# line/Human-Interaction-Generation

Measured on AMD Instinct MI355X. Metric: denoiser-fwd frames/s @ B=64·T=196, higher is better.
Workload: dtype f32; 1 GPU; MotionTransformer forward incl. the per-call cross-attention text side, BASELINE config 2: B=64/GPU T=196 F=150 d=512 L=8 H=8 ff=1024 N=77 Lt=256, linear attention, text embeddings supplied (CLIP stubbed); parallelism=dp1

## Files before the change

human-interaction-generation_amd/csrc/gemm.hip:

```cpp
#include <stdlib.h>

#include "hig_common.h"
#include "hig_host.h"

typedef float f32x16 __attribute__((ext_vector_type(16)));
typedef float f32x4 __attribute__((ext_vector_type(4)));
#ifndef HIG_GEMM_NT
#define HIG_GEMM_NT 0
#endif
#ifndef HIG_GEMM_SETPRIO
#define HIG_GEMM_SETPRIO 1
#endif
#ifndef HIG_GEMM_LDS_EPI
#define HIG_GEMM_LDS_EPI 1
#endif

namespace {

constexpr int BK = 32;
constexpr int NTHREADS = 256;
constexpr int RC_LD = BK + 4;
constexpr int BF_LD = BK + 8;
typedef __bf16 bf16x8 __attribute__((ext_vector_type(8)));
typedef __bf16 bf16x4 __attribute__((ext_vector_type(4)));
// ... 800 lines not shown
      } else {
        a.xsum = g.xcolsum;
      }
    }
  }
  auto al16 = [](const void* p) { return (reinterpret_cast<uintptr_t>(p) & 15) == 0; };
  a.vecx = (g.ldx % 4 == 0) && al16(g.X);
  a.vecy = (g.ldy % 4 == 0) && al16(g.Y);
  a.vecc = (a.g.ldc % 4 == 0) && al16(a.g.C) && (a.slab % 4 == 0) &&
           (!g.res || ((g.ldr % 4 == 0) && al16(g.res))) &&
           (!g.aux || ((g.ldaux % 4 == 0) && al16(g.aux)));
  constexpr int kStage = ((X_RS ? BK * BI : BI * RC_LD) + (Y_RS ? BK * BJ : BJ * RC_LD));
  constexpr int kLdsF32 = 2 * kStage * 4;
  constexpr int kLdsBf3 = 2 * (BI + BJ) * (BF_LD / 2) * 2 * 4;
  const int lds_bytes = (g.prec == HIG_PREC_BF16X3 && !X_RS && !Y_RS) ? kLdsBf3 : kLdsF32;
  int per_cu = 160 * 1024 / lds_bytes;
  per_cu = per_cu < 1 ? 1 : (per_cu > 8 ? 8 : per_cu);
  const int max_vgpr_blocks = (BI * BJ >= 128 * 128) ? 2 : 4;
  if (per_cu > max_vgpr_blocks) per_cu = max_vgpr_blocks;
  const bool fast = hig_gemm32_fast(g);
  if (tail_s > 1) {
    const int rem = a.ntiles % hig_chip_cus();
    a.tail_s = tail_s;
    a.tail_rem = rem;
    a.nmain = a.ntiles - rem;
    a.tail_chunk = g.R / tail_s;
    a.tail_ws = g_tail.ws;
    a.tail_cnt = g_tail.cnt;
    a.ntiles = a.nmain + rem * tail_s;
  }
  int gridx = hig_chip_cus() * per_cu;
  if (gridx > a.ntiles) gridx = a.ntiles;
  bool served = false;
  if constexpr (X_RS && Y_RS && XF == HIG_XF_NONE && EPI == HIG_EPI_NONE) {
    if (splits > 1 && a.g.C == slabs) {
      const int rc = hig_wgrad_wsp32_try(g, splits, slabs, a.slab, a.xsum, a.xsum_stride, st);
      if (rc < 0) return rc;
      served = rc == HIG_OK;
    }
  }
  if (!served && a.ntiles > 0 && g.R >= 0) {
    hig_gemm_path_count(a.tail_s > 1 ? HIG_GEMM_PATH_TAIL32 : splits > 1 ? HIG_GEMM_PATH_SPLIT32 : HIG_GEMM_PATH_TILED32);
    bool launched = false;
    if constexpr (!X_RS && !Y_RS) {
      if (fast && g.prec == HIG_PREC_BF16X3) {
        hipLaunchKernelGGL((gemm_f32_kernel<BI, BJ, X_RS, Y_RS, XF, XF_ON_Y, EPI, true, HIG_PREC_BF16X3>),
                           dim3(gridx, splits), dim3(NTHREADS), 0, st, a);
        launched = true;
      } else if (fast && g.prec == HIG_PREC_BF16) {
        hipLaunchKernelGGL((gemm_f32_kernel<BI, BJ, X_RS, Y_RS, XF, XF_ON_Y, EPI, true, HIG_PREC_BF16>),
                           dim3(gridx, splits), dim3(NTHREADS), 0, st, a);
        launched = true;
      }
    }
    if (!launched) {
      if (fast)
        hipLaunchKernelGGL((gemm_f32_kernel<BI, BJ, X_RS, Y_RS, XF, XF_ON_Y, EPI, true, HIG_PREC_F32>),
                           dim3(gridx, splits), dim3(NTHREADS), 0, st, a);
      else
        hipLaunchKernelGGL((gemm_f32_kernel<BI, BJ, X_RS, Y_RS, XF, XF_ON_Y, EPI, false, HIG_PREC_F32>),
                           dim3(gridx, splits), dim3(NTHREADS), 0, st, a);
    }
  }
  HIG_CHECK_LAUNCH();
  if (splits > 1) {
    const int64_t n4 = (int64_t)g.I * g.J / 4;
    const int64_t want = (n4 + 255) / 256;
    const int blocks = (int)(want > 2048 ? 2048 : want);
    hipLaunchKernelGGL(reduce_slabs_kernel, dim3(blocks), dim3(256), 0, st, slabs, splits, a.slab, n4, g.C,
                       a.xsum ? n4 + g.I / 4 : (int64_t)0, a.xsum ? g.xcolsum : (float*)nullptr, se);
    HIG_CHECK_LAUNCH();
  }
  return HIG_OK;
}

template <bool X_RS, bool Y_RS, int XF, bool XF_ON_Y, int EPI>
int launch_sized(const hig_gemm_desc& g, int splits, float* slabs, int64_t slab, hipStream_t st, const SplitEpilogue& se, int variant) {
  const int tile = splits > 1 ? (wgrad_tile(g.I, g.J, g.prec) == 128 ? 0 : 3) : variant % 16, tail_s = splits > 1 ? 1 : variant / 16;
  switch (tile) {
    case 0: return launch<128, 128, X_RS, Y_RS, XF, XF_ON_Y, EPI>(g, splits, slabs, slab, st, se, tail_s);
    case 1: return launch<64, 128, X_RS, Y_RS, XF, XF_ON_Y, EPI>(g, splits, slabs, slab, st, se, tail_s);
    case 2: return launch<128, 64, X_RS, Y_RS, XF, XF_ON_Y, EPI>(g, splits, slabs, slab, st, se, tail_s);
    default: return launch<64, 64, X_RS, Y_RS, XF, XF_ON_Y, EPI>(g, splits, slabs, slab, st, se, tail_s);
  }
}

}

namespace {
int gemm_dispatch(const hig_gemm_desc& g, int splits, float* slabs, hipStream_t st, const SplitEpilogue& se);
}
int hig_chip_cus() {
  static int cache[64];
  int dev = 0;
  if (hipGetDevice(&dev) != hipSuccess || dev < 0 || dev >= 64) return 256;
  int v = __atomic_load_n(&cache[dev], __ATOMIC_RELAXED);
  if (v == 0) {
    if (hipDeviceGetAttribute(&v, hipDeviceAttributeMultiprocessorCount, dev) != hipSuccess || v <= 0) v = 256;
    static const int forced = getenv("HIG_CHIP_CUS") ? atoi(getenv("HIG_CHIP_CUS")) : 0;
    if (forced > 0) v = forced;
    __atomic_store_n(&cache[dev], v, __ATOMIC_RELAXED);
  }
  return v;
}

int hig_reduce_slabs(const float* slabs, int splits, int64_t slab, int64_t n, float* out, hipStream_t st) {
  const int64_t n4 = n / 4;
  const int64_t want = (n4 + 255) / 256;
  const int blocks = (int)(want > 2048 ? 2048 : (want < 1 ? 1 : want));
  hipLaunchKernelGGL(reduce_slabs_kernel, dim3(blocks), dim3(256), 0, st, slabs, splits, slab, n4, out, (int64_t)0,
                     (float*)nullptr, SplitEpilogue{nullptr, nullptr, 0, 1});
  HIG_CHECK_LAUNCH();
  return HIG_OK;
}

int hig_gemm_launch(const hig_gemm_desc& g, int splits, float* slabs, hipStream_t st) {
  return gemm_dispatch(g, splits, slabs, st, SplitEpilogue{nullptr, nullptr, 0, 1});
}
void hig_gemm_set_tail_scratch(void* ws, int64_t bytes) {
  if (!ws || bytes <= HIG_GEMM_TAIL_CNT_BYTES || (reinterpret_cast<uintptr_t>(ws) & 15)) {
    g_tail = TailScratch{nullptr, nullptr, 0};
    return;
  }
  g_tail.cnt = static_cast<unsigned*>(ws);
  g_tail.ws = reinterpret_cast<float*>(static_cast<char*>(ws) + HIG_GEMM_TAIL_CNT_BYTES);
  g_tail.ws_bytes = bytes - HIG_GEMM_TAIL_CNT_BYTES;
}
namespace {
int gemm_dispatch(const hig_gemm_desc& g, int splits, float* slabs, hipStream_t st, const SplitEpilogue& se) {
  const hig_plan p = hig_gemm32_plan(g, g_tail.ws ? g_tail.ws_bytes : 0, hig_gemm_switch_values(), hig_chip_cus());
  if (p.rc != HIG_OK) return hig_set_error(p.rc, "%s", p.msg);
  if (p.launches == 0) return HIG_OK;
  const int64_t slab = (int64_t)g.I * g.J;
  if (splits > 1) HIG_REQUIRE(slabs && g.epi == HIG_EPI_NONE && slab % 4 == 0 && g.ldc == g.J,
                              "hig_gemm: split-R needs slabs, EPI_NONE, dense C");
  if (splits <= 1 && p.path == HIG_GEMM_PATH_WSP32) {
    if (p.launches == 1) return hig_gemm_wsp32_launch(g, p.variant, st);
    hig_gemm_desc p1, p2;
    hig_gemm32_two_pass(g, &p1, &p2);
    HIG_TRY(hig_gemm_wsp32_launch(p1, p.variant, st));
    return hig_gemm_wsp32_launch(p2, HIG_WSP_VARIANT(0, 0), st);
  }
#define CASE(xrs, yrs, xfv, ony, epiv)                                                   \
  if (g.x_rs == xrs && g.y_rs == yrs && g.xf == xfv && (g.xf == HIG_XF_NONE || g.xf_on_y == ony) && \
      g.epi == epiv)                                                                     \
    return launch_sized<xrs, yrs, xfv, ony, epiv>(g, splits, slabs, slab, st, se, p.variant);
  HIG_GEMM32_COMBOS(CASE)
#undef CASE
  return hig_set_error(HIG_EUNSUPPORTED, "hig_gemm: combination x_rs=%d y_rs=%d xf=%d on_y=%d epi=%d not built",
                       g.x_rs, g.y_rs, g.xf, g.xf_on_y, g.epi);
}
}

int hig_gemm_few_rows(const hig_gemm_desc& g, float* scratch, int64_t scratch_floats, hipStream_t st) {
  const int enabled = hig_gemm_switch_values().few_rows_split;
  const int64_t out = (int64_t)g.I * g.J;
  const bool ok = enabled && scratch && g.I > 0 && g.I <= 64 && g.x_rs == 0 && g.y_rs == 0 && g.ldc == g.J && g.J % 4 == 0 &&
                  (g.epi == HIG_EPI_BIAS || g.epi == HIG_EPI_BIAS_RES) && g.bias &&
                  (g.xf == HIG_XF_NONE || g.xf == HIG_XF_SILU) && g.R % 32 == 0 &&
                  (reinterpret_cast<uintptr_t>(g.bias) & 15) == 0 && (reinterpret_cast<uintptr_t>(g.C) & 15) == 0 &&
                  (g.epi != HIG_EPI_BIAS_RES || (g.res && (reinterpret_cast<uintptr_t>(g.res) & 15) == 0 && g.ldr % 4 == 0));
  int splits = 1;
  if (ok) {
    const int64_t tiles = (g.J + 63) / 64;
    int64_t s = 1024 / tiles;
    if (s > g.R / 64) s = g.R / 64;
    if (s > 16) s = 16;
    if (s * out > scratch_floats) s = scratch_floats / out;
    splits = (int)(s < 1 ? 1 : s);
  }
  if (splits <= 1) return hig_gemm_launch(g, 1, nullptr, st);
  hig_gemm_desc p = g;
  p.epi = HIG_EPI_NONE;
  p.bias = nullptr;
  p.res = nullptr;
  return gemm_dispatch(p, splits, scratch, st,
                       SplitEpilogue{g.bias, g.epi == HIG_EPI_BIAS_RES ? g.res : nullptr, g.ldr, g.J / 4});
}

extern "C" int hig_gemm(const hig_gemm_desc* g, hig_stream_t stream) {
  HIG_REQUIRE(g, "hig_gemm: null descriptor");
  HIG_REQUIRE(g->prec == HIG_PREC_F32 || g->prec == HIG_PREC_BF16X3 || g->prec == HIG_PREC_BF16,
              "hig_gemm: unknown prec %d", g->prec);
  return hig_gemm_launch(*g, 1, nullptr, hig_stream(stream));
}

extern "C" int hig_gemm_debug_stamps(void* buf) {
  g_gemm_stamps = static_cast<unsigned long long*>(buf);
  return HIG_OK;
}

extern "C" int64_t hig_gemm_tail_ws_bytes(void) { return HIG_GEMM_TAIL_BYTES; }

static long long g_path_launches[HIG_GEMM_NPATHS];
void hig_gemm_path_count(int path) {
  if (path >= 0 && path < HIG_GEMM_NPATHS) __atomic_fetch_add(&g_path_launches[path], 1, __ATOMIC_RELAXED);
}
extern "C" int64_t hig_gemm_path_launches(int32_t path) {
  if (path < 0 || path >= HIG_GEMM_NPATHS) return -1;
  return __atomic_load_n(&g_path_launches[path], __ATOMIC_RELAXED);
}

extern "C" int hig_gemm_ws(const hig_gemm_desc* g, void* ws, int64_t ws_bytes, hig_stream_t stream) {
  HIG_REQUIRE(g, "hig_gemm_ws: null descriptor");
  HIG_REQUIRE(g->prec == HIG_PREC_F32 || g->prec == HIG_PREC_BF16X3 || g->prec == HIG_PREC_BF16,
              "hig_gemm_ws: unknown prec %d", g->prec);
  HIG_REQUIRE(!ws || (ws_bytes >= HIG_GEMM_TAIL_BYTES && (reinterpret_cast<uintptr_t>(ws) & 15) == 0),
              "hig_gemm_ws: scratch must be 16-byte aligned and hig_gemm_tail_ws_bytes() long");
  hig_gemm_set_tail_scratch(ws, ws_bytes);
  const int rc = hig_gemm_launch(*g, 1, nullptr, hig_stream(stream));
  hig_gemm_set_tail_scratch(nullptr, 0);
  return rc;
}

extern "C" int64_t hig_gemm_split_scratch_floats(const hig_gemm_desc* g, int32_t splits) {
  if (!g || g->I <= 0 || g->J <= 0) return -1;
  const int64_t per = (int64_t)g->I * g->J + g->I;
  const int64_t cap = splits > 0 ? splits : (g->R / 256 > 1 ? g->R / 256 : 1);
  return per * cap;
}
extern "C" int hig_gemm_split(const hig_gemm_desc* g, int32_t splits, float* slabs, int64_t slab_floats,
                              hig_stream_t stream) {
  HIG_REQUIRE(g && slabs && splits >= 0, "hig_gemm_split: bad arguments");
  HIG_REQUIRE(g->prec == HIG_PREC_F32 || g->prec == HIG_PREC_BF16X3 || g->prec == HIG_PREC_BF16,
              "hig_gemm_split: unknown prec %d", g->prec);
  int s = splits > 0 ? splits : wgrad_splits(g->I, g->J, g->R, slab_floats, g->prec);
  HIG_REQUIRE((int64_t)s * ((int64_t)g->I * g->J + g->I) <= slab_floats, "hig_gemm_split: %d splits need %lld scratch floats, got %lld",
              s, (long long)((int64_t)s * ((int64_t)g->I * g->J + g->I)), (long long)slab_floats);
  return hig_gemm_launch(*g, s, slabs, hig_stream(stream));
}
```

human-interaction-generation_amd/csrc/hig_host.h:

```cpp
#pragma once
#include <stdlib.h>
#include <string.h>

#include <type_traits>

#include "hig_common.h"

int hig_gemm_launch(const hig_gemm_desc& g, int splits, float* slabs, hipStream_t st);
void hig_gemm_path_count(int path);
void hig_attn_path_count(int path, int split);
int hig_gemm_few_rows(const hig_gemm_desc& g, float* scratch, int64_t scratch_floats, hipStream_t st);

constexpr int64_t HIG_GEMM_TAIL_CNT_BYTES = 1024;
constexpr int64_t HIG_GEMM_TAIL_BYTES = HIG_GEMM_TAIL_CNT_BYTES + 256 * 16384;
void hig_gemm_set_tail_scratch(void* ws, int64_t bytes);

int hig_chip_cus();
inline int hig_chip_xcds() { const int c = hig_chip_cus() / 32; return c < 1 ? 1 : c; }

int hig_gemm16_launch(const hig_gemm16_desc& g, hipStream_t st);
int hig_gemm16_split_launch(const hig_gemm16_desc& g, int splits, float* slabs, int64_t slab_floats, hipStream_t st);
struct hig_wg_reduce {
  const float* slabs; int nsplit; int64_t slab;
  int64_t n4; float* out;
  int64_t nb4; float* dbias;
};
constexpr int HIG_WG_RB_MAX = 12;
int hig_wgrad16_launch(const void* dC, int64_t ldd, const void* act, int64_t ldx, int64_t rows, int J, int K, float* dW, float* dbias,
                       int splits, float* slabs, int64_t slab_floats, hipStream_t st, hig_wg_reduce* deferred = nullptr);
int hig_wgrad16_reduce_batch(const hig_wg_reduce* entries, int n, hipStream_t st);
struct hig_wg_problem {
  const void* dC; int64_t ldd; const void* act; int64_t ldx; int64_t rows; int J, K; float* dW; float* dbias; int splits;
};
constexpr int HIG_WG_GROUP_MAX = 4;
int hig_wgrad16_launch_group(const hig_wg_problem* probs, int n, float* slabs, int64_t slab_floats, hipStream_t st, hig_wg_reduce* deferred,
                             int64_t* used_floats);
int64_t hig_wgrad16_rule_floats(int64_t rows, int J, int K, int64_t room);
int hig_reduce_slabs(const float* slabs, int splits, int64_t slab, int64_t n, float* out, hipStream_t st);
struct hig_gemm_switches {
  int wsp16, ws16, ws_rows, ws_nwj, lnfold, lnfold1024, fewrow16, tile16;
  int wsp32, tile32, tail32;
  int few_rows_split;
};
const hig_gemm_switches& hig_gemm_switch_values();
struct hig_plan { int rc, path, launches, variant; char msg[256]; };
#define HIG_WSP_VARIANT(xt, aux) ((xt) + 4 * ((aux) ? 1 : 0))
#define HIG_WS16_VARIANT(nwj, role) ((nwj) + 256 * (role))
#define HIG_TILE16_VARIANT(rows, bk, ns) ((rows) * 1000 + (bk) * 10 + (ns))
#define HIG_TILE32_VARIANT(tile, tail) ((tile) + 16 * (tail))
hig_plan hig_gemm16_plan(const hig_gemm16_desc& g, const hig_gemm_switches& sw, int cus);
hig_plan hig_gemm32_plan(const hig_gemm_desc& g, int64_t tail_ws_bytes, const hig_gemm_switches& sw, int cus);
bool hig_gemm_ws16_lnfold_ok(int64_t rows, int d);
int hig_gemm_wsp16_launch(const hig_gemm16_desc& g, int variant, hipStream_t st);
int hig_gemm_ws16_launch(const hig_gemm16_desc& g, int variant, hipStream_t st);
int hig_gemm_wsp32_launch(const hig_gemm_desc& g, int variant, hipStream_t st);
constexpr int64_t HIG_GEMM_TAIL_UNIT_BYTES = 256 * 16 * 4;
constexpr int HIG_P32_MAXSEG = 3;
inline int hig_wsp32_segments(int np, int* seg_p0, int* seg_np) {
  int nseg = 0, p0 = 0;
  for (int s = 0; s < HIG_P32_MAXSEG; ++s) { seg_p0[s] = 0; seg_np[s] = 1; }
  while (np > 0) {
    int n = 256;
    while (n > np) n >>= 1;
    if (nseg == HIG_P32_MAXSEG) return -1;
    seg_p0[nseg] = p0; seg_np[nseg] = n; ++nseg;
    p0 += n; np -= n;
  }
  return nseg;
}
inline void hig_gemm32_two_pass(const hig_gemm_desc& g, hig_gemm_desc* p1, hig_gemm_desc* p2) {
  *p1 = g; p1->R = 1024;
  *p2 = g; p2->X = g.X + 1024; p2->Y = g.Y + 1024; p2->R = g.R - 1024;
  p2->epi = HIG_EPI_RES; p2->bias = nullptr; p2->res = g.C; p2->ldr = g.ldc;
}
inline bool hig_gemm32_fast(const hig_gemm_desc& g) {
  auto vec = [](const void* p, int64_t ld) { return ld % 4 == 0 && (reinterpret_cast<uintptr_t>(p) & 15) == 0; };
  return vec(g.X, g.ldx) && vec(g.Y, g.ldy) && g.R % 32 == 0 && g.R > 0 && (!g.x_rs || (g.I % 4 == 0 && g.I >= 4)) && (!g.y_rs || (g.J % 4 == 0 && g.J >= 4));
}
#ifdef HIG_GEMM_PROBE
#define HIG_GEMM32_COMBOS(CASE) CASE(0, 0, HIG_XF_NONE, 0, HIG_EPI_BIAS_GELU)
#else
#define HIG_GEMM32_COMBOS(CASE)                                                                                       \
                                                                                \
  CASE(0, 0, HIG_XF_NONE, 0, HIG_EPI_NONE) CASE(0, 0, HIG_XF_NONE, 0, HIG_EPI_BIAS) CASE(0, 0, HIG_XF_NONE, 0, HIG_EPI_BIAS_GELU) \
  CASE(0, 0, HIG_XF_NONE, 0, HIG_EPI_BIAS_POS) CASE(0, 0, HIG_XF_NONE, 0, HIG_EPI_BIAS_RES)                           \
  CASE(0, 0, HIG_XF_NONE, 0, HIG_EPI_RES)                                 \
  CASE(0, 0, HIG_XF_NONE, 0, HIG_EPI_DGELU) CASE(0, 0, HIG_XF_LN, 0, HIG_EPI_BIAS) CASE(0, 0, HIG_XF_LN_MOD_SILU, 0, HIG_EPI_BIAS_RES) \
  CASE(0, 0, HIG_XF_SILU, 0, HIG_EPI_BIAS) CASE(0, 0, HIG_XF_SILU, 0, HIG_EPI_BIAS_RES)                               \
  CASE(0, 0, HIG_XF_SILU, 0, HIG_EPI_NONE)                                 \
                                                                                             \
  CASE(0, 1, HIG_XF_NONE, 0, HIG_EPI_NONE) CASE(0, 1, HIG_XF_NONE, 0, HIG_EPI_RES) CASE(0, 1, HIG_XF_NONE, 0, HIG_EPI_DGELU) \
                                                                                      \
  CASE(1, 1, HIG_XF_NONE, 0, HIG_EPI_NONE) CASE(1, 1, HIG_XF_LN, 1, HIG_EPI_NONE) CASE(1, 1, HIG_XF_LN_MOD_SILU, 1, HIG_EPI_NONE) \
  CASE(1, 1, HIG_XF_SILU, 1, HIG_EPI_NONE)
#endif
template <int... E> struct hig_epi_list {};
using hig_epi16_fewrow = hig_epi_list<HIG_EPI_NONE, HIG_EPI_BIAS, HIG_EPI_BIAS_GELU, HIG_EPI_BIAS_RES, HIG_EPI_BIAS_SILU, HIG_EPI_BIAS_RES_SILU>;
using hig_epi16_all = hig_epi_list<HIG_EPI_NONE, HIG_EPI_BIAS, HIG_EPI_BIAS_GELU, HIG_EPI_BIAS_RES, HIG_EPI_BIAS_SILU, HIG_EPI_BIAS_RES_SILU, HIG_EPI_RES, HIG_EPI_DGELU>;
template <int... E, class F>
int hig_with_epi(hig_epi_list<E...>, int epi, int none, F&& f) {
  int rc = none;
  (void)(((epi == E) && ((rc = f(std::integral_constant<int, E>{})), true)) || ...);
  return rc;
}
struct hig_attn_switches {
  int apply_wave;
  int fullattn_waves;
  int fullattn_valu;
};
const hig_attn_switches& hig_attn_switch_values();
struct hig_attn_call {
  int entry, io;
  int B, rows, Tk, H, hd;
  bool has_scratch;
  int facts;
};
inline int hig_attn_facts(bool operands, uintptr_t in, uintptr_t out, uintptr_t par = 0, bool out_i32 = true) {
  return (operands ? HIG_ATTN_FACT_OPERANDS : 0) | ((in & 7) ? 0 : HIG_ATTN_FACT_IN8) | ((in & 15) ? 0 : HIG_ATTN_FACT_IN16) |
         ((out & 7) ? 0 : HIG_ATTN_FACT_OUT8) | ((out & 15) ? 0 : HIG_ATTN_FACT_OUT16) | ((par & 15) ? 0 : HIG_ATTN_FACT_PAR16) |
         (out_i32 ? HIG_ATTN_FACT_OUT_I32 : 0);
}
inline uintptr_t hig_low_bits(const void* p) { return reinterpret_cast<uintptr_t>(p); }
inline uintptr_t hig_low_bits(int64_t ld, int elem_bytes) { return (uintptr_t)ld * (uintptr_t)elem_bytes; }
struct hig_attn_plan_t { int rc, path, split, variant; char msg[160]; };
#define HIG_ATTN_VARIANT_MERGE 1
hig_attn_plan_t hig_attn_plan_for(const hig_attn_call& c, const hig_attn_switches& sw, int cus, bool big_lds_ok);
bool hig_attn_mfma_hd(int hd);
inline int hig_attn_plan_entry(hig_attn_plan_t* p, const hig_attn_call& c, bool big_lds_ok = true) {
  *p = hig_attn_plan_for(c, hig_attn_switch_values(), hig_chip_cus(), big_lds_ok);
  if (p->rc != HIG_OK) return hig_set_error(p->rc, "%s", p->msg);
  hig_attn_path_count(p->path, p->split);
  return HIG_OK;
}
struct hig_denoiser_switches {
  int32_t text_batch, text_fork, fwd_split, lnfold32, fwd16_fork, ctx16, joint16, fuse_apply, fuse_out, edge16, bwd_overlap;
};
static_assert(sizeof(hig_denoiser_switches) == HIG_DN_NSWITCHES * sizeof(int32_t), "one int32 per switch, in the documented order");
const hig_denoiser_switches& hig_denoiser_switch_values();
struct hig_denoiser_call {
  int entry;
  int B, T, F, d, E, ff, L, H, hd, N, nsty, two, full, prec;
  bool training, has_xf_out;
  int facts;
  bool capturing;
};
struct hig_denoiser_plan_t {
  int32_t entry;
  int32_t text_batched, text_fork, fuse_apply, fold32, split;
  int32_t fork_emb, fork_text, ctx_mm16, joint16, fuse_mm16, fuse_out;
  int32_t fuse_front;
  int32_t wgrad_fork;
  int32_t edge16, Fp;
  int32_t wants_side_stream;
};
static_assert(sizeof(hig_denoiser_plan_t) == HIG_DN_PLAN_NSLOTS * sizeof(int32_t), "one int32 per HIG_DN_PLAN_* slot");
hig_denoiser_plan_t hig_denoiser_plan_for(const hig_denoiser_call& c, const hig_denoiser_switches& sw, int cus, bool wsp32_active);
constexpr int HIG_MAX_TEXT_LAYERS = 32;
struct hig_edge16_offsets { int64_t dout, x, wot, dwo, dwj, dbo, end; };
inline hig_edge16_offsets hig_edge16_layout(int64_t M, int64_t Fp, int d) {
  auto up256 = [](int64_t v) { return (v + 255) / 256 * 256; };
  hig_edge16_offsets e;
  e.dout = 0;
  e.x = e.dout + up256(M * Fp * 2);
  e.wot = e.x + up256(M * Fp * 2);
// ... 146 lines not shown
```

include/hig.h:

```cpp
#ifndef HIG_H
#define HIG_H

#include <stddef.h>
#include <stdint.h>

#ifdef __cplusplus
extern "C" {
#endif

#define HIG_OK 0
#define HIG_EINVAL (-1)
#define HIG_EHIP (-2)
#define HIG_EUNSUPPORTED (-3)

#define HIG_ATTN_LINEAR 0
#define HIG_ATTN_FULL 1

#define HIG_PREC_F32 0
#define HIG_PREC_BF16X3 1
#define HIG_PREC_BF16 2

typedef void* hig_stream_t;

int hig_version(void);
// ... 191 lines not shown

int hig_denoiser_bwd(const hig_dims* dims, const void* const* params, const float* x,
                     const int64_t* t, const int64_t* length, const float* xf_out,
                     const void* textctx, const void* workspace, const float* dout,
                     void* const* grads, float* dx, float* dxf_proj, float* dxf_out,
                     void* bwd_workspace, hig_stream_t stream);
int64_t hig_bwd_workspace_bytes(const hig_dims* dims);
int hig_denoiser_bwd_hooked(const hig_dims* dims, const void* const* params, const float* x,
                            const int64_t* t, const int64_t* length, const float* xf_out,
                            const void* textctx, const void* workspace, const float* dout,
                            void* const* grads, float* dx, float* dxf_proj, float* dxf_out,
                            void* bwd_workspace, hig_stream_t stream, hig_layer_hook hook, void* hook_user,
                            hig_stream_t comm_stream);

typedef struct hig_text_dims {
  int32_t B, N, W;
  int32_t Lt, H, ff, L, E;
  int32_t prec;
} hig_text_dims;
enum {
  HIG_T_PRE_W = 0, HIG_T_PRE_B,
  HIG_T_LN_W, HIG_T_LN_B,
  HIG_T_PROJ_W, HIG_T_PROJ_B,
  HIG_T_NGLOBAL
};
enum {
  HIG_TL_IN_W = 0, HIG_TL_IN_B,
  HIG_TL_OUT_W, HIG_TL_OUT_B,
  HIG_TL_N1_W, HIG_TL_N1_B,
  HIG_TL_FF1_W, HIG_TL_FF1_B,
  HIG_TL_FF2_W, HIG_TL_FF2_B,
  HIG_TL_N2_W, HIG_TL_N2_B,
  HIG_TL_NLAYER
};
int64_t hig_text_head_workspace_bytes(const hig_text_dims* dims, int training);
int64_t hig_text_head_bwd_workspace_bytes(const hig_text_dims* dims);
int hig_text_head_fwd(const hig_text_dims* dims, const void* const* params, const float* clip_out,
                      const int64_t* eot, float* xf_out, float* xf_proj, void* workspace, int training,
                      hig_stream_t stream);
int hig_text_head_bwd(const hig_text_dims* dims, const void* const* params, const float* clip_out,
                      const int64_t* eot, const float* xf_out, const void* workspace, const float* dxf_out,
                      const float* dxf_proj, void* const* grads, float* dclip, void* bwd_workspace,
                      hig_stream_t stream);

enum { HIG_CD_B = 0, HIG_CD_N, HIG_CD_W, HIG_CD_H, HIG_CD_L, HIG_CD_VOCAB, HIG_CD_PREC, HIG_CD_NSLOTS };
enum {
  HIG_CT_TOK_EMB = 0,
  HIG_CT_POS_EMB,
  HIG_CT_LNF_W, HIG_CT_LNF_B,
  HIG_CT_NGLOBAL
};
enum {
  HIG_CTL_LN1_W = 0, HIG_CTL_LN1_B,
  HIG_CTL_IN_W, HIG_CTL_IN_B,
  HIG_CTL_OUT_W, HIG_CTL_OUT_B,
  HIG_CTL_LN2_W, HIG_CTL_LN2_B,
  HIG_CTL_FC_W, HIG_CTL_FC_B,
  HIG_CTL_PROJ_W, HIG_CTL_PROJ_B,
  HIG_CTL_NLAYER
};
int64_t hig_clip_text_workspace_bytes(const int32_t* dims);
int hig_clip_text_fwd(const int32_t* dims, const void* const* params, const int64_t* tokens, float* out,
                      void* workspace, hig_stream_t stream);
int hig_clip_embed(const float* tok_emb, const float* pos_emb, const int64_t* tokens, int32_t B, int32_t N, int32_t W,
                   int32_t vocab, float* out, int64_t ldo, hig_stream_t stream);
int hig_quick_gelu(float* x, int64_t n, hig_stream_t stream);
int hig_causal_attn_fwd(const float* Q, int64_t ldq, const float* K, const float* V, int64_t ldk, int32_t B, int32_t N,
                        int32_t H, float* Y, int64_t ldy, hig_stream_t stream);

typedef struct hig_eval_dims {
  int32_t B, T, F;
  int32_t d, H, ff, L;
  int32_t C;
  int32_t cls;
  int32_t prec;
} hig_eval_dims;
enum {
  HIG_EV_SEQ_EMB = 0,
  HIG_EV_JOINT1_W, HIG_EV_JOINT1_B,
  HIG_EV_JOINT2_W, HIG_EV_JOINT2_B,
  HIG_EV_OUT1_W, HIG_EV_OUT1_B,
  HIG_EV_OUT2_W, HIG_EV_OUT2_B,
  HIG_EV_HEAD_W, HIG_EV_HEAD_B,
  HIG_EV_CLS_IN,
  HIG_EV_NGLOBAL
};
int64_t hig_eval_encoder_workspace_bytes(const hig_eval_dims* dims);
int hig_eval_encoder_fwd(const hig_eval_dims* dims, const void* const* params, const float* x1,
                         const float* x2, const int64_t* length, float* logits, float* feature,
                         void* workspace, hig_stream_t stream);
int64_t hig_eval_encoder_train_workspace_bytes(const hig_eval_dims* dims);
int64_t hig_eval_encoder_bwd_workspace_bytes(const hig_eval_dims* dims);
int hig_eval_encoder_fwd_train(const hig_eval_dims* dims, const void* const* params, const float* x1,
                               const float* x2, const int64_t* length, float* logits, float* feature,
                               void* workspace, hig_stream_t stream);
int hig_eval_encoder_bwd(const hig_eval_dims* dims, const void* const* params, const float* x1, const float* x2,
                         const int64_t* length, const void* workspace, const float* dlogits,
                         const float* dfeature , void* const* grads, void* bwd_workspace,
                         hig_stream_t stream);
int hig_softmax_xent(const float* logits, const int64_t* labels, int32_t B, int32_t C, float* loss ,
                     float* dlogits, int64_t* pred, hig_stream_t stream);

int hig_gather_frames(const float* bank, const int64_t* seq_off, const int32_t* frame_ix,
                      const void* stats, int32_t stats_f64, int32_t rows, int32_t T, int32_t F,
                      float* out, hig_stream_t stream);

int hig_eval_pairs_build(const float* src, const int64_t* src_off, const int32_t* m_len, const int32_t* shift,
                         const int64_t* src_off_host, const int32_t* m_len_host, const int32_t* shift_host,
                         int64_t src_floats, int32_t N, int32_t F_in, int32_t F_out, int32_t T_out, float* out,
                         hig_stream_t stream);

int hig_recover_joints(const float* motion, const float* stats, int32_t rows, int32_t T, int32_t F,
                       int32_t joints, int32_t init_first, float* pos, hig_stream_t stream);


#define HIG_XF_NONE 0
#define HIG_XF_LN 1
#define HIG_XF_LN_MOD_SILU 2
#define HIG_XF_SILU 3
#define HIG_EPI_NONE 0
#define HIG_EPI_BIAS 1
#define HIG_EPI_BIAS_GELU 2
#define HIG_EPI_BIAS_RES 3
#define HIG_EPI_BIAS_POS 4
#define HIG_EPI_RES 5
#define HIG_EPI_DGELU 6
#define HIG_EPI_BIAS_SILU 7
#define HIG_EPI_BIAS_RES_SILU 8
typedef struct hig_gemm_desc {
  const float* X; int64_t ldx; int32_t x_rs;
  const float* Y; int64_t ldy; int32_t y_rs;
  float* C; int64_t ldc;
  int32_t I, J, R;
  int32_t xf, xf_on_y, epi, prec;
  const float* bias;
  const float* res; int64_t ldr;
  float* aux; int64_t ldaux;
  const float* stats;
  const float* gamma; const float* beta;
  const float* ss; int64_t ss_ld; int32_t ss_shift_off; int32_t rows_per_sample;
  const float* pos; int64_t ldpos; int32_t T;
  int32_t pos_shift;
  float* xcolsum;
  float* row_stats_out;
  const float* row_stats_in;
  const float* ln_colsum;
} hig_gemm_desc;
int hig_gemm(const hig_gemm_desc* g, hig_stream_t stream);
int64_t hig_gemm_tail_ws_bytes(void);
int hig_gemm_ws(const hig_gemm_desc* g, void* ws, int64_t ws_bytes, hig_stream_t stream);
int hig_gemm_debug_stamps(void* buf);
int64_t hig_gemm_split_scratch_floats(const hig_gemm_desc* g, int32_t splits);
int hig_gemm_split(const hig_gemm_desc* g, int32_t splits, float* slabs, int64_t slab_floats, hig_stream_t stream);

typedef struct hig_gemm16_desc {
  const void* X; int64_t ldx;
  const void* Y; int64_t ldy;
  void* C; int64_t ldc; int32_t c_f32;
  int32_t I, J, R;
  int32_t epi;
  const float* bias;
  const void* res; int64_t ldr; int32_t res_f32;
  float* row_stats_out;
  const float* row_stats_in;
  const float* ln_colsum;
  void* aux; int64_t ldaux;
} hig_gemm16_desc;
int hig_gemm_bf16(const hig_gemm16_desc* g, hig_stream_t stream);
int64_t hig_gemm_bf16_split_scratch_floats(const hig_gemm16_desc* g, int32_t splits);
int hig_gemm_bf16_split(const hig_gemm16_desc* g, int32_t splits, float* slabs, int64_t slab_floats, hig_stream_t stream);
int hig_gemm_bf16_debug_stamps(void* buf);
int hig_gemm_ws16_debug_stamps(void* buf);
int hig_gemm_wsp16_debug_stamps(void* buf);
int hig_gemm_wsp32_debug_stamps(void* buf);
int64_t hig_gemm_wsp32_launches(void);
#define HIG_GEMM_PATH_TILED32 0
#define HIG_GEMM_PATH_WSP32 1
#define HIG_GEMM_PATH_TAIL32 2
#define HIG_GEMM_PATH_WGRAD_WSP32 3
#define HIG_GEMM_PATH_SPLIT32 4
#define HIG_GEMM_PATH_WSP16 5
#define HIG_GEMM_PATH_WS16 6
#define HIG_GEMM_PATH_FEWROW16 7
#define HIG_GEMM_PATH_TILED16 8
#define HIG_GEMM_PATH_SPLIT16 9
#define HIG_GEMM_PATH_WGRAD16 10
#define HIG_GEMM_NPATHS 11
int64_t hig_gemm_path_launches(int32_t path);
int hig_gemm_bf16_plan(const hig_gemm16_desc* g, int32_t chip_cus, int32_t* path, int32_t* launches, int32_t* variant);
int hig_gemm_plan(const hig_gemm_desc* g, int32_t has_tail_scratch, int32_t chip_cus, int32_t* path, int32_t* launches, int32_t* variant);
int hig_gemm_bf16_lnfold_plan(int64_t rows, int32_t d, int32_t chip_cus);
#define HIG_ATTN_PATH_CTX 0
#define HIG_ATTN_PATH_CTX_MFMA 1
#define HIG_ATTN_PATH_CTX_PART 2
#define HIG_ATTN_PATH_APPLY 3
#define HIG_ATTN_PATH_APPLY_MFMA 4
#define HIG_ATTN_PATH_APPLY_WAVE64 5
#define HIG_ATTN_PATH_APPLY_STY 6
#define HIG_ATTN_PATH_APPLY_STY_WAVE64 7
#define HIG_ATTN_PATH_APPLY_BWD 8
#define HIG_ATTN_PATH_APPLY_BWD_MFMA 9
#define HIG_ATTN_PATH_CTX_BWD 10
#define HIG_ATTN_PATH_CTX_BWD_MFMA 11
#define HIG_ATTN_PATH_FULL_FWD 12
#define HIG_ATTN_PATH_FULL_FWD_MFMA 13
#define HIG_ATTN_PATH_FULL_BWD 14
#define HIG_ATTN_PATH_FULL_BWD_MFMA 15
#define HIG_ATTN_NPATHS 16
int64_t hig_attn_path_launches(int32_t path);
int32_t hig_attn_last_split(void);
#define HIG_ATTN_ENTRY_CTX 0
#define HIG_ATTN_ENTRY_APPLY 1
#define HIG_ATTN_ENTRY_APPLY_STY 2
#define HIG_ATTN_ENTRY_APPLY_BWD 3
#define HIG_ATTN_ENTRY_CTX_BWD 4
#define HIG_ATTN_ENTRY_FULL_FWD 5
#define HIG_ATTN_ENTRY_FULL_BWD 6
#define HIG_ATTN_IO_F32 0
#define HIG_ATTN_IO_BF16 1
#define HIG_ATTN_FACT_IN8 1
#define HIG_ATTN_FACT_IN16 2
#define HIG_ATTN_FACT_OUT8 4
#define HIG_ATTN_FACT_OUT16 8
#define HIG_ATTN_FACT_PAR16 16
#define HIG_ATTN_FACT_OUT_I32 32
#define HIG_ATTN_FACT_OPERANDS 64
#define HIG_ATTN_FACTS_ALL 127
int hig_attn_plan(int32_t entry, int32_t io, int32_t B, int32_t rows, int32_t Tk, int32_t H, int32_t hd, int32_t has_scratch,
                  int32_t facts, int32_t chip_cus, int32_t big_lds_ok, int32_t* path, int32_t* split, int32_t* variant);
#define HIG_DN_ENTRY_TEXT32 0
#define HIG_DN_ENTRY_TEXT16 1
#define HIG_DN_ENTRY_FWD32 2
#define HIG_DN_ENTRY_FWD16 3
#define HIG_DN_ENTRY_FWD16_TRAIN 4
#define HIG_DN_ENTRY_BWD32 5
#define HIG_DN_ENTRY_BWD16 6
#define HIG_DN_FACT_TABLE 1
#define HIG_DN_FACT_TEXT_GLOBALS 2
#define HIG_DN_FACT_KVALL 4
#define HIG_DN_NSWITCHES 11
#define HIG_DN_PLAN_ENTRY 0
#define HIG_DN_PLAN_TEXT_BATCHED 1
#define HIG_DN_PLAN_TEXT_FORK 2
#define HIG_DN_PLAN_FUSE_APPLY 3
#define HIG_DN_PLAN_FOLD32 4
#define HIG_DN_PLAN_SPLIT 5
#define HIG_DN_PLAN_FORK_EMB 6
#define HIG_DN_PLAN_FORK_TEXT 7
#define HIG_DN_PLAN_CTX_MM16 8
#define HIG_DN_PLAN_JOINT16 9
#define HIG_DN_PLAN_FUSE_MM16 10
#define HIG_DN_PLAN_FUSE_OUT 11
#define HIG_DN_PLAN_FUSE_FRONT 12
#define HIG_DN_PLAN_WGRAD_FORK 13
#define HIG_DN_PLAN_EDGE16 14
#define HIG_DN_PLAN_FP 15
#define HIG_DN_PLAN_WANTS_SIDE_STREAM 16
#define HIG_DN_PLAN_NSLOTS 17
int hig_denoiser_plan(const hig_dims* dims, int32_t entry, int32_t training, int32_t has_xf_out, int32_t derived_facts, int32_t capturing,
                      int32_t chip_cus, int32_t wsp32_active, const int32_t* switches, int32_t* out, int32_t n_out);
int32_t hig_denoiser_last_schedule(int32_t* out, int32_t n_out);
int hig_wgrad16_debug_stamps(void* buf);
int hig_linattn16_debug_stamps(void* buf);
#define HIG_LAYOUT16_FWD 0
#define HIG_LAYOUT16_TEXT 1
#define HIG_LAYOUT16_BWD 2
#define HIG_LAYOUT16_TAP 3
enum {
  HIG_FW16_TE = 0, HIG_FW16_TE_H, HIG_FW16_EMB, HIG_FW16_SS, HIG_FW16_H0, HIG_FW16_TOK0, HIG_FW16_LENP, HIG_FW16_LAYER0, HIG_FW16_LSTRIDE,
  HIG_FW16_XN1, HIG_FW16_QKV, HIG_FW16_A1, HIG_FW16_AT1, HIG_FW16_KST1, HIG_FW16_Y1, HIG_FW16_A1S, HIG_FW16_H1, HIG_FW16_XN2, HIG_FW16_QC,
  HIG_FW16_Y2, HIG_FW16_A2S, HIG_FW16_H2, HIG_FW16_Z1, HIG_FW16_F1, HIG_FW16_Y3, HIG_FW16_A3S, HIG_FW16_H3, HIG_FW16_XN3, HIG_FW16_IQKV,
  HIG_FW16_AI, HIG_FW16_ATI, HIG_FW16_KSTI, HIG_FW16_Y4, HIG_FW16_A4S, HIG_FW16_H2B, HIG_FW16_TOTAL, HIG_FW16_NSLOTS
};
enum { HIG_TX16_LAYER0 = 0, HIG_TX16_LSTRIDE, HIG_TX16_XFN, HIG_TX16_KV, HIG_TX16_AC, HIG_TX16_ATC, HIG_TX16_KSTC, HIG_TX16_TOTAL, HIG_TX16_NSLOTS };
enum { HIG_BW16_DSS = 0, HIG_BW16_DEMB, HIG_BW16_DTE_H, HIG_BW16_MP, HIG_BW16_MTP, HIG_BW16_TOTAL, HIG_BW16_NSLOTS };
enum {
  HIG_TAP16_DHL = 0, HIG_TAP16_DTMP_EMB, HIG_TAP16_DEMB, HIG_TAP16_DTMP_TE, HIG_TAP16_DTE_H, HIG_TAP16_DSS, HIG_TAP16_TOK0, HIG_TAP16_POSTMP,
  HIG_TAP16_LAYER0, HIG_TAP16_LSTRIDE,
  HIG_TAP16_DH_IN, HIG_TAP16_FFN_T1, HIG_TAP16_FFN_DY, HIG_TAP16_FFN_DZ, HIG_TAP16_FFN_DH,
  HIG_TAP16_INT_T1, HIG_TAP16_INT_DY, HIG_TAP16_INT_DQKV, HIG_TAP16_INT_DA, HIG_TAP16_INT_T2, HIG_TAP16_INT_DH,
  HIG_TAP16_CA_T1, HIG_TAP16_CA_DY, HIG_TAP16_CA_DQ, HIG_TAP16_CA_DA, HIG_TAP16_CA_T2, HIG_TAP16_CA_DH, HIG_TAP16_CA_DKV, HIG_TAP16_CA_DXFN,
  HIG_TAP16_CA_DXF_OUT,
  HIG_TAP16_SA_T1, HIG_TAP16_SA_DY, HIG_TAP16_SA_DQKV, HIG_TAP16_SA_DA, HIG_TAP16_SA_T2, HIG_TAP16_SA_DH,
  HIG_TAP16_TOTAL, HIG_TAP16_NSLOTS
};
int hig_bf16_train_layout(const hig_dims* dims, int32_t which, int64_t* out, int32_t n_out);
int hig_denoiser_bwd_bf16_debug_tap(void* buf, int64_t bytes);
int64_t hig_denoiser_bwd_bf16_tap_bytes(const hig_dims* dims);
int64_t hig_joint_embed_bf16_scratch_bytes(int32_t F, int32_t d);
int hig_joint_embed_bf16_w(const float* x, int64_t M, int32_t F, const void* w_padded, const float* bias, const float* pos,
                           int64_t ldpos, int32_t T, int32_t pos_shift, void* out, int64_t ldo, int32_t d, hig_stream_t stream);
int hig_joint_embed_bf16(const float* x, int64_t M, int32_t F, const float* W, const float* bias, const float* pos,
                         int64_t ldpos, int32_t T, int32_t pos_shift, void* out, int64_t ldo, int32_t d,
                         void* w_scratch, hig_stream_t stream);
int hig_cast_bf16(const float* src, void* dst, int64_t n, hig_stream_t stream);

int hig_ln_bf16(const void* x, int32_t x_f32, int64_t ldx, int64_t rows, int32_t n, const float* gamma,
                const float* beta, const float* ss, int64_t ss_ld, int32_t ss_shift_off, int32_t rows_per_sample,
                void* out, int64_t ldo, hig_stream_t stream);
int hig_linattn_ctx_bf16(const void* K, const void* V, int64_t ld, int32_t B, int32_t rows, int32_t H, int32_t hd,
                         const int64_t* length, float* A, float* kstat, float* scratch, void* At16, hig_stream_t stream);
int hig_linattn_apply_bf16(const void* Q, int64_t ldq, const float* A, void* Y, int64_t ldy, int32_t B, int32_t rows,
                           int32_t H, int32_t hd, hig_stream_t stream);
int hig_linattn_ctx_mm16(const void* K, const void* V, int64_t ld, int32_t B, int32_t rows, int32_t H, int32_t hd,
                         const int64_t* length, float* A, float* kstat, void* At16, hig_stream_t stream);
int hig_linattn_apply_sty_bf16(const void* Q, int64_t ldq, const float* A, const float* gamma, const float* beta,
// ... 154 lines not shown
```

Baseline: 2.148 million frames/s.

## Add single-launch intra-block split-K fp32 GEMM for few-row matmuls

Adds a dedicated fp32 MFMA kernel for GEMMs with at most 64 rows (such as the timestep or condition projections). It splits the K dimension across the four waves of a block, reduces their partials in LDS, and applies bias, residual and optional SiLU in one launch. This replaces the split-K path that wrote slabs to scratch and needed a separate reduction. It is on whenever the few_rows switch is enabled and not set to 2, and it adds a public entry point that takes an explicit mode.

After: 2.148 million frames/s. Within noise of the previous version (-0.0%).

```diff
diff --git a/human-interaction-generation_amd/csrc/gemm.hip b/human-interaction-generation_amd/csrc/gemm.hip
--- a/human-interaction-generation_amd/csrc/gemm.hip
+++ b/human-interaction-generation_amd/csrc/gemm.hip
@@ -976,8 +976,15 @@
 }
 }
 
+namespace {
+int few_rows(const hig_gemm_desc& g, int enabled, float* scratch, int64_t scratch_floats, hipStream_t st);
+}
 int hig_gemm_few_rows(const hig_gemm_desc& g, float* scratch, int64_t scratch_floats, hipStream_t st) {
-  const int enabled = hig_gemm_switch_values().few_rows_split;
+  return few_rows(g, hig_gemm_switch_values().few_rows_split, scratch, scratch_floats, st);
+}
+namespace {
+int few_rows(const hig_gemm_desc& g, int enabled, float* scratch, int64_t scratch_floats, hipStream_t st) {
+  if (enabled && enabled != 2 && hig_gemm_fewrow32_serves(g)) return hig_gemm_fewrow32_launch(g, st);
   const int64_t out = (int64_t)g.I * g.J;
   const bool ok = enabled && scratch && g.I > 0 && g.I <= 64 && g.x_rs == 0 && g.y_rs == 0 && g.ldc == g.J && g.J % 4 == 0 &&
                   (g.epi == HIG_EPI_BIAS || g.epi == HIG_EPI_BIAS_RES) && g.bias &&
@@ -1001,12 +1008,21 @@
   return gemm_dispatch(p, splits, scratch, st,
                        SplitEpilogue{g.bias, g.epi == HIG_EPI_BIAS_RES ? g.res : nullptr, g.ldr, g.J / 4});
 }
+}
 
 extern "C" int hig_gemm(const hig_gemm_desc* g, hig_stream_t stream) {
   HIG_REQUIRE(g, "hig_gemm: null descriptor");
   HIG_REQUIRE(g->prec == HIG_PREC_F32 || g->prec == HIG_PREC_BF16X3 || g->prec == HIG_PREC_BF16,
               "hig_gemm: unknown prec %d", g->prec);
   return hig_gemm_launch(*g, 1, nullptr, hig_stream(stream));
+}
+
+extern "C" int hig_gemm_few_rows_call(const hig_gemm_desc* g, int32_t mode, float* scratch, int64_t scratch_floats, hig_stream_t stream) {
+  HIG_REQUIRE(g, "hig_gemm_few_rows_call: null descriptor");
+  HIG_REQUIRE(g->prec == HIG_PREC_F32 || g->prec == HIG_PREC_BF16X3 || g->prec == HIG_PREC_BF16,
+              "hig_gemm_few_rows_call: unknown prec %d", g->prec);
+  HIG_REQUIRE(scratch_floats >= 0 && (scratch || scratch_floats == 0), "hig_gemm_few_rows_call: bad scratch");
+  return few_rows(*g, mode < 0 ? hig_gemm_switch_values().few_rows_split : mode, scratch, scratch_floats, hig_stream(stream));
 }
 
 extern "C" int hig_gemm_debug_stamps(void* buf) {
diff --git a/human-interaction-generation_amd/csrc/gemm_fewrow32.hip b/human-interaction-generation_amd/csrc/gemm_fewrow32.hip
--- /dev/null
+++ b/human-interaction-generation_amd/csrc/gemm_fewrow32.hip
@@ -0,0 +1,174 @@
+#include "hig_common.h"
+#include "hig_host.h"
+
+namespace {
+
+typedef float f32x4 __attribute__((ext_vector_type(4)));
+
+constexpr int FR_WAVES = 4;
+constexpr int fr_lds_bytes(int rt, int ct) { return FR_WAVES * 16 * (rt + ct) * 128; }
+
+__device__ __forceinline__ float fr_silu(float x) {
+  return x * __builtin_amdgcn_rcpf(1.0f + __builtin_amdgcn_exp2f(x * -1.4426950408889634f));
+}
+
+template <int RT, int CT, int DEPTH, bool SILU>
+__global__ __launch_bounds__(FR_WAVES * 64) void gemm_fewrow32_kernel(const float* __restrict__ X, int64_t ldx,
+                                                                      const float* __restrict__ W, int64_t ldy,
+                                                                      float* __restrict__ C, int64_t ldc, int I, int J, int R,
+                                                                      const float* __restrict__ bias, const float* __restrict__ res,
+                                                                      int64_t ldr) {
+  constexpr int ROWS = 16 * RT, XL = 2 * RT, WL = 2 * CT;
+  constexpr int EG = CT < 3 ? CT : 3, EW = 16 * EG;
+  static_assert(CT % EG == 0, "panel = whole epilogue groups");
+  static_assert(FR_WAVES * ROWS * EW * 4 <= fr_lds_bytes(RT, CT), "the partial sums fit the operand images");
+  extern __shared__ __attribute__((aligned(16))) float fr_lds[];
+  const int tid = threadIdx.x, w = tid >> 6, l = tid & 63;
+  const int r8 = l >> 3, p8 = l & 7;
+  const int r16 = l & 15, q = l >> 4;
+  const int j0 = blockIdx.x * (16 * CT), i0 = blockIdx.y * ROWS;
+  float* img = fr_lds + w * (16 * (RT + CT) * 32);
+
+  const float* xp[XL];
+  const float* wp[WL];
+#pragma unroll
+  for (int g = 0; g < XL; ++g) xp[g] = X + (int64_t)min(i0 + g * 8 + r8, I - 1) * ldx + p8 * 4;
+#pragma unroll
+  for (int g = 0; g < WL; ++g) wp[g] = W + (int64_t)min(j0 + g * 8 + r8, J - 1) * ldy + p8 * 4;
+  const int wo[2] = {r8 * 32 + 4 * (p8 ^ (r8 >> 1)), r8 * 32 + 4 * (p8 ^ ((r8 >> 1) | 4))};
+  const int ro[2] = {r16 * 32 + 4 * ((2 * q) ^ (r16 >> 1)), r16 * 32 + 4 * ((2 * q + 1) ^ (r16 >> 1))};
+
+  f32x4 acc[RT][CT];
+#pragma unroll
+  for (int rt = 0; rt < RT; ++rt)
+#pragma unroll
+    for (int ct = 0; ct < CT; ++ct) acc[rt][ct] = f32x4{0.f, 0.f, 0.f, 0.f};
+
+  const int npieces = R / 32;
+  const int nmine = (npieces - w + FR_WAVES - 1) / FR_WAVES;
+  const int nlast = nmine > 0 ? nmine - 1 : 0;
+
+  f32x4 xv[DEPTH][XL], wv[DEPTH][WL];
+  auto fetch = [&](int slot, int n) {
+    const int off = (nmine > 0 ? w + FR_WAVES * min(n, nlast) : 0) * 32;
+#pragma unroll
+    for (int g = 0; g < WL; ++g) wv[slot][g] = *reinterpret_cast<const f32x4*>(wp[g] + off);
+#pragma unroll
+    for (int g = 0; g < XL; ++g) xv[slot][g] = *reinterpret_cast<const f32x4*>(xp[g] + off);
+  };
+#pragma unroll
+  for (int p = 0; p < DEPTH; ++p) fetch(p, p);
+
+  auto multiply = [&](f32x4 (&xs)[XL], const f32x4 (&ws)[WL]) {
+#pragma unroll
+    for (int g = 0; g < XL; ++g) {
+      if (SILU) {
+#pragma unroll
+        for (int s = 0; s < 4; ++s) xs[g][s] = fr_silu(xs[g][s]);
+      }
+      *reinterpret_cast<f32x4*>(img + g * 256 + wo[g & 1]) = xs[g];
+    }
+#pragma unroll
+    for (int g = 0; g < WL; ++g) *reinterpret_cast<f32x4*>(img + (XL + g) * 256 + wo[g & 1]) = ws[g];
+    asm volatile("s_waitcnt lgkmcnt(0)" ::: "memory");
+    __builtin_amdgcn_wave_barrier();
+#pragma unroll
+    for (int u = 0; u < 2; ++u) {
+      f32x4 a[RT], b[CT];
+#pragma unroll
+      for (int rt = 0; rt < RT; ++rt) a[rt] = *reinterpret_cast<const f32x4*>(img + rt * 512 + ro[u]);
+#pragma unroll
+      for (int ct = 0; ct < CT; ++ct) b[ct] = *reinterpret_cast<const f32x4*>(img + (RT + ct) * 512 + ro[u]);
+#pragma unroll
+      for (int s = 0; s < 4; ++s)
+#pragma unroll
+        for (int rt = 0; rt < RT; ++rt)
+#pragma unroll
+          for (int ct = 0; ct < CT; ++ct)
+            acc[rt][ct] = __builtin_amdgcn_mfma_f32_16x16x4f32(a[rt][s], b[ct][s], acc[rt][ct], 0, 0, 0);
+    }
+    asm volatile("" ::: "memory");
+    __builtin_amdgcn_wave_barrier();
+  };
+  int n0 = 0;
+  for (; n0 + DEPTH <= nmine; n0 += DEPTH) {
+#pragma unroll
+    for (int p = 0; p < DEPTH; ++p) {
+      multiply(xv[p], wv[p]);
+      __builtin_amdgcn_sched_barrier(0);
+      fetch(p, n0 + p + DEPTH);
+      __builtin_amdgcn_sched_barrier(0);
+    }
+  }
+#pragma unroll
+  for (int p = 0; p < DEPTH - 1; ++p) {
+    if (n0 + p < nmine) multiply(xv[p], wv[p]);
+  }
+
+  float* red = fr_lds;
+  constexpr int EW4 = EW / 4;
+#pragma unroll
+  for (int h = 0; h < CT / EG; ++h) {
+    __syncthreads();
+#pragma unroll
+    for (int rt = 0; rt < RT; ++rt)
+#pragma unroll
+      for (int c = 0; c < EG; ++c)
+#pragma unroll
+        for (int e = 0; e < 4; ++e) red[(w * ROWS + rt * 16 + q * 4 + e) * EW + c * 16 + r16] = acc[rt][h * EG + c][e];
+    __syncthreads();
+    for (int v = tid; v < ROWS * EW4; v += FR_WAVES * 64) {
+      const int i = v / EW4, jj = 4 * (v - i * EW4), j = j0 + h * EW + jj;
+      if (i0 + i >= I || j >= J) continue;
+      f32x4 s = *reinterpret_cast<const f32x4*>(&red[i * EW + jj]);
+#pragma unroll
+      for (int k = 1; k < FR_WAVES; ++k) s += *reinterpret_cast<const f32x4*>(&red[(k * ROWS + i) * EW + jj]);
+      s += *reinterpret_cast<const f32x4*>(bias + j);
+      if (res) s += *reinterpret_cast<const f32x4*>(res + (int64_t)(i0 + i) * ldr + j);
+      *reinterpret_cast<f32x4*>(C + (int64_t)(i0 + i) * ldc + j) = s;
+    }
+  }
+}
+
+template <int RT, int CT, int DEPTH>
+int launch_fewrow32(const hig_gemm_desc& g, hipStream_t st) {
+  constexpr int lds = fr_lds_bytes(RT, CT);
+  static const int lds_rc = [] {
+    if (lds <= 64 * 1024) return 0;
+    return hipFuncSetAttribute(reinterpret_cast<const void*>(&gemm_fewrow32_kernel<RT, CT, DEPTH, true>), hipFuncAttributeMaxDynamicSharedMemorySize, lds) == hipSuccess &&
+           hipFuncSetAttribute(reinterpret_cast<const void*>(&gemm_fewrow32_kernel<RT, CT, DEPTH, false>), hipFuncAttributeMaxDynamicSharedMemorySize, lds) == hipSuccess ? 0 : 1;
+  }();
+  if (lds_rc != 0) return hig_set_error(HIG_EHIP, "gemm_fewrow32: cannot reserve %d bytes of LDS", lds);
+  const dim3 grid((g.J + 16 * CT - 1) / (16 * CT), (g.I + 16 * RT - 1) / (16 * RT));
+  const float* res = g.epi == HIG_EPI_BIAS_RES ? g.res : nullptr;
+  if (g.xf == HIG_XF_SILU)
+    hipLaunchKernelGGL((gemm_fewrow32_kernel<RT, CT, DEPTH, true>), grid, dim3(FR_WAVES * 64), lds, st, g.X, g.ldx, g.Y, g.ldy, g.C, g.ldc,
+                       g.I, g.J, g.R, g.bias, res, g.ldr);
+  else
+    hipLaunchKernelGGL((gemm_fewrow32_kernel<RT, CT, DEPTH, false>), grid, dim3(FR_WAVES * 64), lds, st, g.X, g.ldx, g.Y, g.ldy, g.C, g.ldc,
+                       g.I, g.J, g.R, g.bias, res, g.ldr);
+  HIG_CHECK_LAUNCH();
+  return HIG_OK;
+}
+
+}
+
+bool hig_gemm_fewrow32_serves(const hig_gemm_desc& g) {
+  const auto al16 = [](const void* p) { return (reinterpret_cast<uintptr_t>(p) & 15) == 0; };
+  return g.prec == HIG_PREC_F32 && g.X && g.Y && g.C && g.I > 0 && g.I <= 64 && g.J > 0 && g.J % 4 == 0 && g.R > 0 && g.R % 32 == 0 &&
+         g.x_rs == 0 && g.y_rs == 0 && g.ldc == g.J && g.ldx % 4 == 0 && g.ldy % 4 == 0 && g.ldx >= g.R && g.ldy >= g.R &&
+         (g.xf == HIG_XF_NONE || (g.xf == HIG_XF_SILU && !g.xf_on_y)) && (g.epi == HIG_EPI_BIAS || g.epi == HIG_EPI_BIAS_RES) &&
+         g.bias && al16(g.bias) && al16(g.C) && al16(g.X) && al16(g.Y) && !g.aux && !g.xcolsum && !g.row_stats_out && !g.row_stats_in &&
+         !g.ln_colsum && (g.epi != HIG_EPI_BIAS_RES || (g.res && al16(g.res) && g.ldr % 4 == 0 && g.ldr >= g.J));
+}
+
+int hig_gemm_fewrow32_launch(const hig_gemm_desc& g, hipStream_t st) {
+  HIG_REQUIRE(hig_gemm_fewrow32_serves(g), "gemm_fewrow32: not served (I %d J %d R %d xf %d epi %d)", g.I, g.J, g.R, g.xf, g.epi);
+  if ((g.J + 47) / 48 < hig_chip_cus()) return launch_fewrow32<1, 1, 4>(g, st);
+  switch ((g.I + 15) / 16) {
+    case 1: return launch_fewrow32<1, 3, 2>(g, st);
+    case 2: return launch_fewrow32<2, 3, 2>(g, st);
+    case 3: return launch_fewrow32<3, 3, 2>(g, st);
+    default: return launch_fewrow32<4, 3, 2>(g, st);
+  }
+}
diff --git a/human-interaction-generation_amd/csrc/hig_host.h b/human-interaction-generation_amd/csrc/hig_host.h
--- a/human-interaction-generation_amd/csrc/hig_host.h
+++ b/human-interaction-generation_amd/csrc/hig_host.h
@@ -10,6 +10,8 @@
 void hig_gemm_path_count(int path);
 void hig_attn_path_count(int path, int split);
 int hig_gemm_few_rows(const hig_gemm_desc& g, float* scratch, int64_t scratch_floats, hipStream_t st);
+bool hig_gemm_fewrow32_serves(const hig_gemm_desc& g);
+int hig_gemm_fewrow32_launch(const hig_gemm_desc& g, hipStream_t st);
 
 constexpr int64_t HIG_GEMM_TAIL_CNT_BYTES = 1024;
 constexpr int64_t HIG_GEMM_TAIL_BYTES = HIG_GEMM_TAIL_CNT_BYTES + 256 * 16384;
diff --git a/include/hig.h b/include/hig.h
--- a/include/hig.h
+++ b/include/hig.h
@@ -367,6 +367,7 @@
 int hig_gemm_debug_stamps(void* buf);
 int64_t hig_gemm_split_scratch_floats(const hig_gemm_desc* g, int32_t splits);
 int hig_gemm_split(const hig_gemm_desc* g, int32_t splits, float* slabs, int64_t slab_floats, hig_stream_t stream);
+int hig_gemm_few_rows_call(const hig_gemm_desc* g, int32_t mode, float* scratch, int64_t scratch_floats, hig_stream_t stream);
 
 typedef struct hig_gemm16_desc {
   const void* X; int64_t ldx;
```
